# UltimateSoftware/surge

Hardware: AMD Instinct MI355X
Metric: events/sec replayed (higher is better)
Workload: dtype int32/int64 adds + bit-copied f64

## Files before the change

surge_amd/csrc/ingest_decoder.hip:

```cpp
#include <cstdio>
#include <cstdlib>

#include "ingest_decoder_internal.h"

using namespace surge::ingest;
using namespace surge::ingest::host;

namespace {

struct DecoderOptions {
  int push_streams = 3;
  bool push_streams_pinned = false, normal_priority = false, block_waits = true, weak_hash = false;
  int64_t poll_ns = 10000;
};

DecoderOptions read_options() {
  DecoderOptions o;
  if (const char* v = std::getenv("SURGE_INGEST_PUSH_STREAMS")) {
    o.push_streams = std::atoi(v);
    o.push_streams_pinned = true;
  }
  o.push_streams = o.push_streams < 1 ? 1 : (o.push_streams > kSlots ? kSlots : o.push_streams);
  if (const char* v = std::getenv("SURGE_INGEST_PUSH_PRIORITY")) o.normal_priority = std::strcmp(v, "normal") == 0;
  if (const char* v = std::getenv("SURGE_INGEST_WAIT")) {
    o.block_waits = std::strcmp(v, "spin") != 0;
    if (std::strcmp(v, "poll") != 0) o.poll_ns = 0;
  }
  if (o.poll_ns > 0)
    if (const char* u = std::getenv("SURGE_INGEST_POLL_US")) o.poll_ns = std::atoll(u) > 0 ? std::atoll(u) * 1000 : o.poll_ns;
  if (const char* v = std::getenv("SURGE_INGEST_DEBUG_WEAK_HASH")) o.weak_hash = v[0] == '1';
  return o;
}

int32_t create_streams_and_events(surge_device_decoder* d, const DecoderOptions& o) {
  d->push_streams_pinned = o.push_streams_pinned;
  for (int i = 0; i < o.push_streams; ++i) {
    int least = 0, greatest = 0;
    if (!o.normal_priority && hipDeviceGetStreamPriorityRange(&least, &greatest) == hipSuccess && least != greatest)
      DCHK(d, hipStreamCreateWithPriority(&d->push_streams[i], hipStreamNonBlocking, least));
    else
      DCHK(d, hipStreamCreateWithFlags(&d->push_streams[i], hipStreamNonBlocking));
    d->n_push_streams = d->n_push_active = i + 1;
  }
  for (PushSlot& s : d->slots) {
    DCHK(d, hipEventCreateWithFlags(&s.done, hipEventDisableTiming));
    DCHK(d, hipEventCreateWithFlags(&s.released, hipEventDisableTiming));
    DCHK(d, s.d_err.reserve(sizeof(ErrorCell), false, d->stream));
  }
  DCHK(d, hipEventCreateWithFlags(&d->ready, hipEventDisableTiming));
  DCHK(d, hipEventCreateWithFlags(&d->consumed, hipEventDisableTiming));
  return OK;
}

int32_t upload_template(surge_device_decoder* d, const surge_event_json_template* tmpl) {
  static EvjDevice ev;
  static std::mutex ev_mu;
  std::lock_guard<std::mutex> lk(ev_mu);
  std::memset(&ev, 0, sizeof(ev));
  ev.n_types = tmpl->n_types;
  auto intern = [&](const char* name) -> uint8_t {
// ... 70 lines not shown
    *rc = refuse_poisoned(d);
    return nullptr;
  }
  PushSlot* s = nullptr;
  {
    std::lock_guard<std::mutex> lk(d->mu);
    if (d->n_pending < kSlots) s = &d->slots[(d->head + d->n_pending) % kSlots];
    if (s) s->stream = d->push_streams[d->push_seq++ % (uint64_t)d->n_push_active];
  }
  if (!s) *rc = dfail(d, SURGE_E_STATE, "every push slot holds an unfinished push: call surge_device_decoder_push_finish first");
  return s;
}

int32_t await_release(surge_device_decoder* d, PushSlot& s) {
  if (!s.released_valid) return OK;
  DCHK(d, hipStreamWaitEvent(s.stream, s.released, 0));
  s.released_valid = false;
  return OK;
}

int32_t commit_slot(surge_device_decoder* d, PushSlot& s) {
  DCHK(d, hipEventRecord(s.done, s.stream));
  s.busy = true;
  std::lock_guard<std::mutex> lk(d->mu);
  ++d->n_pending;
  return OK;
}

template <typename Stage1>
int32_t enqueue_push(surge_device_decoder* d, Stage1 stage1) {
  int32_t rc = OK;
  PushSlot* s = claim_slot(d, &rc);
  if (!s) return rc;
  rc = await_release(d, *s);
  if (rc != OK) return rc;
  rc = stage1(*s);
  if (rc != OK) {
    (void)hipStreamSynchronize(s->stream);
    return rc;
  }
  return commit_slot(d, *s);
}

int32_t finish_oldest(surge_device_decoder* d, bool wait) {
  PushSlot* sp;
  {
    std::lock_guard<std::mutex> lk(d->mu);
    if (d->n_pending == 0) sp = nullptr;
    else sp = &d->slots[d->head];
  }
  if (!sp) return dfail(d, SURGE_E_STATE, "push_finish without a pending push_async");
  PushSlot& s = *sp;
  const int32_t rc = stage2(d, s, wait);
  if (rc != OK) {
    (void)hipStreamSynchronize(s.stream);
    (void)hipStreamSynchronize(d->stream);
    s.released_valid = false;
  }
  s.busy = false;
  std::lock_guard<std::mutex> lk(d->mu);
  d->head = (d->head + 1) % kSlots;
  --d->n_pending;
  return rc;
}

void* pinned_alloc(size_t n) {
  void* p = nullptr;
  return hipHostMalloc(&p, n, hipHostMallocDefault) == hipSuccess ? p : nullptr;
}
// ... 27 lines not shown
  return decoder_create(device_id, hip_stream, tmpl, false, out);
}

int32_t surge_device_decoder_create_states(int32_t device_id, void* hip_stream, surge_device_decoder** out) {
  return decoder_create(device_id, hip_stream, nullptr, true, out);
}

int32_t surge_device_decoder_destroy(surge_device_decoder* d) {
  if (!d) return OK;
#ifdef SURGE_EXPERIMENTS
  std::fprintf(stderr, "[surge experiments] decoder: %lld pushes, %lld batches chained by the one-lane walk after the parallel recognition declined\n", (long long)d->pushes,
               (long long)d->chain_fallbacks);
#endif
  DeviceScope scope(d->device);
  (void)hipStreamSynchronize(d->stream);
  for (int i = 0; i < d->n_push_streams; ++i) {
    (void)hipStreamSynchronize(d->push_streams[i]);
    (void)hipStreamDestroy(d->push_streams[i]);
  }
  for (PushSlot& s : d->slots) {
    if (s.done) (void)hipEventDestroy(s.done);
    if (s.released) (void)hipEventDestroy(s.released);
  }
  if (d->ready) (void)hipEventDestroy(d->ready);
  if (d->consumed) (void)hipEventDestroy(d->consumed);
  if (d->sleeper) (void)hipEventDestroy(d->sleeper);
  delete d;
  return OK;
}

int32_t surge_device_decoder_push_parts_floored_async(surge_device_decoder* d, int32_t n_parts, const uint8_t* const* bytes, const surge_batch_section* const* sections,
                                                      const int64_t* n_sections, int64_t n_floors, const surge_section_floor* floors) {
  if (!d) return refuse_null_decoder();
  if (n_parts < 0 || (n_parts > 0 && (!bytes || !sections || !n_sections)) || n_floors < 0 || (n_floors > 0 && !floors)) return dfail(d, E_INVALID, "bad argument");
  DeviceScope scope(d->device);
  return enqueue_push(d, [&](PushSlot& s) { return stage1_wire(d, s, n_parts, bytes, sections, n_sections, n_floors, floors); });
// ... 166 lines not shown
```

surge_amd/csrc/ingest_decoder_internal.h:

```cpp
#pragma once

#include <sys/prctl.h>
#include <time.h>

#include <atomic>
#include <cstring>
#include <mutex>
#include <new>
#include <string>
#include <utility>
#include <vector>

#include "../../include/surge_ingest.h"
#include "../../include/surge_replay.h"
#include "ingest_device.h"

namespace surge {
namespace ingest {
namespace host __attribute__((visibility("hidden"))) {

constexpr int32_t OK = 0, E_INVALID = -1, E_DEVICE = -3, E_NOMEM = -4, E_UNSUPPORTED = -5;

struct Buf {
  void* p = nullptr;
  size_t cap = 0;
  Buf() = default;
  Buf(const Buf&) = delete;
  Buf& operator=(const Buf&) = delete;
  Buf(Buf&& o) noexcept : p(o.p), cap(o.cap) { o.p = nullptr; o.cap = 0; }
  Buf& operator=(Buf&& o) noexcept {
// ... 10 lines not shown
    if (e != hipSuccess) return e;
    if (keep && p && cap) {
      e = hipMemcpyAsync(fresh, p, cap, hipMemcpyDeviceToDevice, stream);
      if (e == hipSuccess) e = hipStreamSynchronize(stream);
      if (e != hipSuccess) { (void)hipFree(fresh); return e; }
    }
    if (p) (void)hipFree(p);
    p = fresh;
    cap = want;
    return hipSuccess;
  }
  void release() { if (p) (void)hipFree(p); p = nullptr; cap = 0; }
};

struct PushSlot {
  Buf lz4_blocks, lz4_sizes, lz4_nseq, lz4_seq, lz4_cls;
  Buf sn_blocks, sn_sizes, sn_nseq, sn_seq, sn_cls;
  Buf d_bytes, d_sections, rec_a, rec_b, rec_c, meta, ev_tmp, f64_list, d_err;
  void* pinned = nullptr;
  size_t pinned_cap = 0;
  std::vector<Section> h_secs;
  Lz4Plan lz4;
  Lz4Plan snappy;
  int64_t snappy_host_sections = 0;
  std::vector<CrcSpan> h_crc;
  Buf crc_spans;
  std::vector<int64_t> h_floors;
  Buf d_floors;
  ErrorCell h_err;
  hipStream_t stream = nullptr;
  hipEvent_t done = nullptr;
  hipEvent_t released = nullptr;
  bool released_valid = false;
  int64_t n_rec = 0;
  uint64_t seed = 0;
  bool busy = false, wire = false;
  ~PushSlot() { if (pinned) (void)hipHostFree(pinned); }
};
constexpr int kSlots = 5;

struct ReadsState {
  struct Lookup { Buf ids, off, idx; } lookup;
  struct Order {
    Buf idx;
    int64_t keys = -1, passes = 0;
  } order;
// ... 61 lines not shown
  bool json = false;
  bool states = false;
  bool continued = false;
  bool keep_strings = false;
  std::mutex mu;
  std::atomic<bool> poisoned{false};
  std::string err;
  Buf d_tmpl, d_ptab;
  surge_event_json_template h_tmpl;
  PushSlot slots[kSlots];
  hipStream_t push_streams[kSlots] = {nullptr, nullptr, nullptr, nullptr, nullptr};
  int n_push_streams = 0;
  int n_push_active = 0;
  bool push_streams_pinned = false;
  uint64_t push_seq = 0;
  int head = 0;
  std::atomic<int> n_pending{0};
  Buf first, first_scan, keep, keep_pos, temp;
  Buf vlen, vscan, val_src, long_runs;
  Buf st_status, st_spans;
  Buf t_slots, arena, key_off, key_hash;
  uint64_t t_cap = 0;
  std::atomic<uint64_t> seed{0};
  int64_t n_keys = 0, arena_bytes = 0;
  Buf r_agg, r_ev, r_off;
  Buf r_val, r_val_off;
  int64_t val_bytes = 0;
  int64_t n_records = 0;
  int64_t state_loads = 0;
  uint64_t events_from_push = 0;
// ... 78 lines not shown
}

inline hipError_t wait_stream(surge_device_decoder* d, hipStream_t st) {
  if (!d->block_waits) return hipStreamSynchronize(st);
  hipError_t e = hipEventRecord(d->sleeper, st);
  if (e != hipSuccess || d->poll_ns <= 0) return e != hipSuccess ? e : hipEventSynchronize(d->sleeper);
  const int slack = prctl(PR_GET_TIMERSLACK, 0, 0, 0, 0);
  if (slack > 1000) (void)prctl(PR_SET_TIMERSLACK, 1000ul, 0, 0, 0);
  const timespec nap{0, (long)d->poll_ns};
  while ((e = hipEventQuery(d->sleeper)) == hipErrorNotReady) (void)nanosleep(&nap, nullptr);
  (void)hipGetLastError();
  if (slack > 1000) (void)prctl(PR_SET_TIMERSLACK, (unsigned long)slack, 0, 0, 0);
  return e;
}

int32_t stage1_wire(surge_device_decoder* d, PushSlot& s, int32_t n_parts, const uint8_t* const* bytes, const surge_batch_section* const* sections,
                    const int64_t* n_sections, int64_t n_floors, const surge_section_floor* floors);
int32_t stage1_records(surge_device_decoder* d, PushSlot& s, const uint8_t* keys, const int64_t* key_off, const uint8_t* values, const int64_t* value_off,
                       const int64_t* offsets, int64_t n);
int32_t stage2(surge_device_decoder* d, PushSlot& s, bool wait);
int32_t merge_event_strings(surge_device_decoder* d);
int32_t merge_state_strings(surge_device_decoder* d, surge_replay_handle* h, const surge_json_template* tmpl);

}
}
}
```

surge_amd/csrc/ingest_device.h:

```cpp
#pragma once

#include <hip/hip_runtime.h>
#include <stdint.h>

#include <vector>

#include "../../include/surge_ingest.h"
#include "f64_parse.h"

namespace surge {
namespace ingest {

enum : uint32_t {
  RS_OK = 0,
  RS_SKIP = 1,
  RS_NULL = 2,
  RS_MALFORMED = 3,
  RS_JSON = 4,
  RS_TYPE = 5,
  RS_FIELD = 6,
  RS_SIZE = 7,
  RS_F64_HOST = 8,
  RS_COLLISION = 9,
  RS_EMPTY_VALUE = 10,
// ... 150 lines not shown
  int64_t n_keys, arena_bytes;
};

struct InternScratch {
  unsigned long long *first, *first_scan;
  uint32_t *keep, *keep_pos;
  void* temp;
  size_t temp_bytes;
};

hipError_t launch_crc(const uint8_t* bytes, const CrcSpan* spans, int32_t n_spans, ErrorCell* err, hipStream_t st);

Lz4Route lz4_plan_section(Lz4Plan& plan, const uint8_t* frame, int64_t frame_len, int64_t src_off, int32_t section, int64_t* area_off,
                          std::vector<uint8_t>& host_out);
Lz4ScratchBytes lz4_scratch_bytes(const Lz4Plan& plan);
hipError_t launch_lz4(const Lz4Plan& plan, const uint8_t* bytes, uint8_t* area, const Lz4Block* d_blocks, Lz4Work w, Section* sections, ErrorCell* err, hipStream_t st);

hipError_t launch_lz4_exec(const uint8_t* bytes, uint8_t* area, const Lz4Block* d_blocks, int64_t n_blocks, Lz4Work w, hipStream_t st);

Lz4Route snappy_plan_section(Lz4Plan& plan, const uint8_t* sec, int64_t len, int64_t src_off, int32_t section, int64_t* area_off, std::vector<uint8_t>& host_out,
                             const char** why);
hipError_t launch_snappy(const Lz4Plan& plan, const uint8_t* bytes, uint8_t* area, const Lz4Block* d_blocks, Lz4Work w, Section* sections, ErrorCell* err, hipStream_t st);

hipError_t launch_sections(const uint8_t* bytes, const Section* sections, int64_t n_sections, int32_t max_recs, uint64_t seed, JsonCtx jc, RecMeta* meta,
                           uint4* ev_tmp, uint32_t* f64_host_list, ErrorCell* err, const int64_t* floors, hipStream_t st);
hipError_t launch_records(const uint8_t* bytes, const int64_t* key_off, const int64_t* val_off, const int64_t* offsets, int64_t val_base, int64_t n_rec,
                          uint64_t seed, JsonCtx jc, RecMeta* meta, uint4* ev_tmp, uint32_t* f64_host_list, ErrorCell* err, hipStream_t st);

hipError_t intern_temp_bytes(int64_t n_rec, size_t* bytes, hipStream_t st);
void launch_table_build(const KeyTable& k, hipStream_t st);
// ... 81 lines not shown
```

surge_amd/csrc/ingest_lz4.hip:

```cpp
#include <new>

#include "ingest_device.h"

namespace surge {
namespace ingest {
namespace {

constexpr int kLz4BlockMax = 65536;
struct Lz4Window {
  const uint8_t* in;
  int32_t n_in, wbase;
  uint32_t win;
  int lane;
  __device__ void refill(int32_t at) {
    wbase = at;
    const int32_t pos = at + 4 * lane;
    uint32_t v = 0;
    if (pos + 4 <= n_in) {
      v = (uint32_t)in[pos] | ((uint32_t)in[pos + 1] << 8) | ((uint32_t)in[pos + 2] << 16) | ((uint32_t)in[pos + 3] << 24);
    } else {
      for (int k = 0; k < 4; ++k)
        if (pos + k < n_in) v |= (uint32_t)in[pos + k] << (8 * k);
    }
    win = v;
// ... 442 lines not shown
  n.seq = (size_t)(plan.n_seq + 1) * 8;
  n.cls = (size_t)(kLz4Classes + 1) * (nb + 1) * 4;
  return n;
}

hipError_t launch_lz4_exec(const uint8_t* bytes, uint8_t* area, const Lz4Block* d_blocks, int64_t nb, Lz4Work w, hipStream_t st) {
  for (int c = 0; c <= kLz4Classes; ++c) {
    const int32_t cap = c < kLz4Classes ? kLz4ClassCapHost[c] : 0;
    const size_t lds = cap ? (size_t)cap + (size_t)kLz4Map * 2 : 0;
    const int64_t resident = 256ll * (lds ? (int64_t)(160 * 1024 / lds) : 16);
    hipLaunchKernelGGL(lz4_exec_kernel, dim3((unsigned)(nb < resident ? nb : resident)), dim3(64), lds, st, bytes, area, d_blocks, (int32_t)nb, w, c, cap);
  }
  return hipGetLastError();
}

hipError_t launch_lz4(const Lz4Plan& plan, const uint8_t* bytes, uint8_t* area, const Lz4Block* d_blocks, Lz4Work w, Section* sections, ErrorCell* err,
                      hipStream_t st) {
  const int64_t nb = (int64_t)plan.blocks.size();
  if (nb == 0) return hipSuccess;
  w.cls_list = w.cls_count + (kLz4Classes + 1);
  const hipError_t e = hipMemsetAsync(w.cls_count, 0, (kLz4Classes + 1) * 4, st);
  if (e != hipSuccess) return e;
  const int32_t parse_caps[3] = {6656, 16384 + 64, kLz4BlockMax + 64};
  for (int c = 0; c < 3; ++c)
    hipLaunchKernelGGL(lz4_parse_kernel, dim3((unsigned)nb), dim3(64), (size_t)parse_caps[c], st, bytes, area, d_blocks, (int32_t)nb, w, sections, err,
                       c == 0 ? -1 : parse_caps[c - 1], parse_caps[c]);
  (void)launch_lz4_exec(bytes, area, d_blocks, nb, w, st);
  bool any_one_pass = false;
  for (const Lz4Block& b : plan.blocks) any_one_pass = any_one_pass || b.seq_off < 0;
  if (any_one_pass) {
    const unsigned grid = (unsigned)(nb < 8192 ? nb : 8192);
    const int32_t caps[3] = {16384, 32768, kLz4BlockMax};
    for (int c = 0; c < 3; ++c)
      hipLaunchKernelGGL(lz4_block_kernel, dim3(grid), dim3(64), (size_t)caps[c], st, bytes, area, d_blocks, nb, w.state, c, caps[c], sections, err);
  }
  return hipGetLastError();
}
// ... 4 lines not shown
```

surge_amd/csrc/ingest_snappy.hip:

```cpp
#include <new>

#include "ingest_device.h"
#include "snappy_block.h"

namespace surge {
namespace ingest {
namespace {

constexpr int32_t kSnappyChunkMax = 65536;
constexpr int kSnappyParseClasses = 4;
constexpr int32_t kSnappyParseCap[kSnappyParseClasses] = {10240, 20480, 40960, 81920};
constexpr int32_t kSnappyStagePad = 80;
constexpr int32_t kSnappyStageMax = kSnappyParseCap[kSnappyParseClasses - 1] - 15 - kSnappyStagePad;
constexpr int32_t kSnappyShortLiteral = 16;

__device__ __forceinline__ int32_t wave_inclusive_sum(int32_t v, int lane) {
#pragma unroll
  for (int d = 1; d < 64; d <<= 1) {
    const int32_t u = __shfl_up(v, d, 64);
    if (lane >= d) v += u;
  }
  return v;
}

// ... 156 lines not shown
    host_out.resize(ex + (size_t)total);
    int64_t got = 0;
    st = sn::frame_decompress(sec, len, host_out.data() + ex, total, &got);
    if (st == sn::SN_OK) return LZ4_ON_HOST;
    host_out.resize(ex);
  }
  *why = sn::status_name(st);
  return st == sn::SN_TOO_LARGE ? LZ4_TOO_LARGE : LZ4_BAD_FRAME;
}

hipError_t launch_snappy(const Lz4Plan& plan, const uint8_t* bytes, uint8_t* area, const Lz4Block* d_blocks, Lz4Work w, Section* sections, ErrorCell* err,
                         hipStream_t st) {
  const int64_t nb = (int64_t)plan.blocks.size();
  if (nb == 0) return hipSuccess;
  w.cls_list = w.cls_count + (kLz4Classes + 1);
  const hipError_t e = hipMemsetAsync(w.cls_count, 0, (kLz4Classes + 1) * 4, st);
  if (e != hipSuccess) return e;
  for (int c = 0; c < kSnappyParseClasses; ++c)
    hipLaunchKernelGGL(snappy_parse_kernel, dim3((unsigned)nb), dim3(64), (size_t)kSnappyParseCap[c], st, bytes, area, d_blocks, (int32_t)nb, w, sections, err,
                       c == 0 ? -1 : kSnappyParseCap[c - 1], kSnappyParseCap[c]);
  return launch_lz4_exec(bytes, area, d_blocks, nb, w, st);
}

}
}
```

surge_amd/csrc/ingest_stage1.hip:

```cpp
#include <chrono>
#include <cstdio>
#include <cstdlib>

#include "ingest_decoder_internal.h"

using namespace surge::ingest;
using namespace surge::ingest::host;

namespace {

int32_t slot_scratch(surge_device_decoder* d, PushSlot& s, int64_t n_rec) {
  const size_t R = (size_t)n_rec;
  DCHK(d, s.meta.reserve(R * sizeof(RecMeta), false, s.stream));
  if (!d->states) DCHK(d, s.ev_tmp.reserve(R * 16, false, s.stream));
  if (!d->states) DCHK(d, s.f64_list.reserve(R * 4, false, s.stream));
  static const ErrorCell kZero{~0ull, 0u, 0u, ~0u, ~0u, 0u, ~0u};
  DCHK(d, hipMemcpyAsync(s.d_err.p, &kZero, sizeof(kZero), hipMemcpyHostToDevice, s.stream));
  return OK;
}

int32_t slot_pinned(surge_device_decoder* d, PushSlot& s, size_t bytes) {
  if (bytes <= s.pinned_cap) return OK;
  if (s.pinned) (void)hipHostFree(s.pinned);
  s.pinned = nullptr;
  s.pinned_cap = 0;
  bytes += bytes / 4 + 65536;
  DCHK(d, hipHostMalloc(&s.pinned, bytes, hipHostMallocDefault));
  s.pinned_cap = bytes;
  return OK;
}

int32_t dbg_decode() {
// ... 26 lines not shown
};

struct WireLayout {
  struct Part {
    int64_t lo, len, dev;
    bool in_place;
  };
  std::vector<Part> parts;
  std::vector<uint8_t> extra;
  int64_t total_sections = 0, n_rec = 0, n_raw = 0;
  int32_t max_recs = 0;
  int64_t area_base() const { return (n_raw + (int64_t)extra.size() + 15) & ~15ll; }
};

struct SlotNeeds {
  size_t bytes, sections, crc_spans, floors, pinned;
  int64_t n_rec;
  Lz4ScratchBytes lz4, snappy;
};

size_t pad16(size_t n) { return (n + 15) & ~(size_t)15; }

constexpr int64_t kSnappyMark = -(1ll << 62);

int32_t layout_sections(surge_device_decoder* d, PushSlot& s, int32_t n_parts, const surge_batch_section* const* sections, const int64_t* n_sections, WireLayout& L) {
  try {
    s.h_secs.resize((size_t)L.total_sections);
    L.parts.resize((size_t)n_parts);
  } catch (const std::bad_alloc&) {
    return dfail(d, E_NOMEM, "out of host memory");
  }
  int64_t at = 0;
  for (int32_t p = 0; p < n_parts; ++p) {
    int64_t lo = INT64_MAX, hi = 0;
// ... 82 lines not shown
  } catch (const std::bad_alloc&) {
    return dfail(d, E_NOMEM, "out of host memory");
  }
  if (s.lz4.blocks.size() >= (1ull << 31)) return dfail(d, E_UNSUPPORTED, "more than 2^31 LZ4 blocks in one push: push fewer sections at a time");
  if (s.snappy.blocks.size() >= (1ull << 31)) return dfail(d, E_UNSUPPORTED, "more than 2^31 snappy chunks in one push: push fewer sections at a time");
  for (Section& sc : s.h_secs) {
    if (sc.byte_off <= kSnappyMark) sc.byte_off = L.area_base() + s.lz4.area + (kSnappyMark - sc.byte_off);
    else if (sc.byte_off < 0) sc.byte_off = L.area_base() + (-1 - sc.byte_off);
  }
  return OK;
}

SlotNeeds slot_needs(const PushSlot& s, const uint8_t* const* bytes, WireLayout& L) {
  SlotNeeds n;
  n.bytes = (size_t)(L.area_base() + s.lz4.area + s.snappy.area) + 64;
  n.sections = sizeof(Section) * s.h_secs.size();
  n.crc_spans = sizeof(CrcSpan) * s.h_crc.size();
  n.n_rec = L.n_rec;
  n.lz4 = lz4_scratch_bytes(s.lz4);
  n.snappy = lz4_scratch_bytes(s.snappy);
  n.floors = 8 * s.h_floors.size();
  n.pinned = pad16(L.extra.size()) + n.sections + n.lz4.blocks + pad16(n.snappy.blocks) + pad16(n.crc_spans) + pad16(n.floors) + 64;
  for (size_t p = 0; p < L.parts.size(); ++p) {
    WireLayout::Part& part = L.parts[p];
    if (part.len == 0) continue;
    hipPointerAttribute_t attr;
    part.in_place = hipPointerGetAttributes(&attr, bytes[p] + part.lo) == hipSuccess && attr.type == hipMemoryTypeHost;
    (void)hipGetLastError();
    if (!part.in_place) n.pinned += pad16((size_t)part.len);
  }
  return n;
}

int32_t size_slot(surge_device_decoder* d, PushSlot& t, const SlotNeeds& n) {
  const size_t per_event = d->states ? 0 : (size_t)n.n_rec;
  const std::pair<Buf*, size_t> device[] = {{&t.d_bytes, n.bytes}, {&t.d_sections, n.sections}, {&t.meta, (size_t)n.n_rec * sizeof(RecMeta)}, {&t.ev_tmp, per_event * 16},
                                            {&t.f64_list, per_event * 4}, {&t.crc_spans, n.crc_spans}, {&t.d_floors, n.floors}, {&t.lz4_blocks, n.lz4.blocks}, {&t.lz4_sizes, n.lz4.state},
                                            {&t.lz4_nseq, n.lz4.n_seq}, {&t.lz4_seq, n.lz4.seq}, {&t.lz4_cls, n.lz4.cls}, {&t.sn_blocks, n.snappy.blocks},
                                            {&t.sn_sizes, n.snappy.state}, {&t.sn_nseq, n.snappy.n_seq}, {&t.sn_seq, n.snappy.seq}, {&t.sn_cls, n.snappy.cls}};
  for (const auto& b : device) DCHK(d, b.first->reserve(b.second, false, t.stream));
  return slot_pinned(d, t, n.pinned);
}

void warm_idle_slots(surge_device_decoder* d, PushSlot& s, const SlotNeeds& n) {
  if (d->slots_sized) return;
  d->slots_sized = true;
  {
    std::lock_guard<std::mutex> lk(d->mu);
    if (d->n_pending != 0) return;
  }
  for (PushSlot& t : d->slots)
    if (&t != &s && !t.busy && !t.released_valid && size_slot(d, t, n) != OK) (void)hipGetLastError();
}

int32_t stage_and_copy(surge_device_decoder* d, PushSlot& s, const uint8_t* const* bytes, const WireLayout& L) {
  hipStream_t st = s.stream;
  size_t staged = 0;
  auto stage = [&](const void* src, size_t len) -> const uint8_t* {
    uint8_t* at = (uint8_t*)s.pinned + staged;
    std::memcpy(at, src, len);
    staged += pad16(len);
    return at;
  };
  for (size_t p = 0; p < L.parts.size(); ++p) {
    const WireLayout::Part& part = L.parts[p];
    if (part.len == 0) continue;
    const uint8_t* src = bytes[p] + part.lo;
    if (!part.in_place) src = stage(src, (size_t)part.len);
    DCHK(d, hipMemcpyAsync((uint8_t*)s.d_bytes.p + part.dev, src, (size_t)part.len, hipMemcpyHostToDevice, st));
  }
  if (!L.extra.empty()) DCHK(d, hipMemcpyAsync((uint8_t*)s.d_bytes.p + L.n_raw, stage(L.extra.data(), L.extra.size()), L.extra.size(), hipMemcpyHostToDevice, st));
  const size_t sec_bytes = sizeof(Section) * s.h_secs.size(), crc_bytes = sizeof(CrcSpan) * s.h_crc.size(), blk_bytes = sizeof(Lz4Block) * s.lz4.blocks.size();
  DCHK(d, hipMemcpyAsync(s.d_sections.p, stage(s.h_secs.data(), sec_bytes), sec_bytes, hipMemcpyHostToDevice, st));
  if (crc_bytes) DCHK(d, hipMemcpyAsync(s.crc_spans.p, stage(s.h_crc.data(), crc_bytes), crc_bytes, hipMemcpyHostToDevice, st));
  if (blk_bytes) DCHK(d, hipMemcpyAsync(s.lz4_blocks.p, stage(s.lz4.blocks.data(), blk_bytes), blk_bytes, hipMemcpyHostToDevice, st));
  const size_t sn_bytes = sizeof(Lz4Block) * s.snappy.blocks.size();
  if (sn_bytes) DCHK(d, hipMemcpyAsync(s.sn_blocks.p, stage(s.snappy.blocks.data(), sn_bytes), sn_bytes, hipMemcpyHostToDevice, st));
  const size_t floor_bytes = 8 * s.h_floors.size();
  if (floor_bytes) DCHK(d, hipMemcpyAsync(s.d_floors.p, stage(s.h_floors.data(), floor_bytes), floor_bytes, hipMemcpyHostToDevice, st));
  return OK;
}

int32_t expand_floors(surge_device_decoder* d, PushSlot& s, int64_t total_sections, int64_t n_floors, const surge_section_floor* floors) {
  s.h_floors.clear();
  if (n_floors == 0) return OK;
  if (d->states) return dfail(d, SURGE_E_STATE, "a state decoder reads its topic from the beginning: floors belong to an events decoder");
  try {
    s.h_floors.assign((size_t)total_sections, INT64_MIN);
  } catch (const std::bad_alloc&) {
    return dfail(d, E_NOMEM, "out of host memory");
  }
  for (int64_t i = 0; i < n_floors; ++i) {
    if (floors[i].section < 0 || floors[i].section >= total_sections) return dfail(d, E_INVALID, "a floor names section " + std::to_string(floors[i].section) + ": the push has " + std::to_string(total_sections));
    int64_t& f = s.h_floors[(size_t)floors[i].section];
// ... 16 lines not shown
  s.n_rec = 0;
  s.wire = true;
  s.snappy.clear();
  s.snappy_host_sections = 0;
  if (L.total_sections >= (1ll << 31)) return dfail(d, E_UNSUPPORTED, "more than 2^31 batches in one push");
  int32_t rc = expand_floors(d, s, L.total_sections, n_floors, floors);
  if (rc != OK || L.total_sections == 0) return rc;
  rc = layout_sections(d, s, n_parts, sections, n_sections, L);
  if (rc != OK || L.n_rec == 0) return rc;
  if (L.n_rec >= (1ll << 32) - 1) return dfail(d, E_UNSUPPORTED, "more than 2^32 - 2 records in one push: push fewer sections at a time");
  rc = plan_frames(d, s, n_parts, bytes, sections, n_sections, L);
  if (rc != OK) return rc;
  laps.lap("walk sections");
  const SlotNeeds needs = slot_needs(s, bytes, L);
  warm_idle_slots(d, s, needs);
  rc = size_slot(d, s, needs);
  if (rc == OK) rc = slot_scratch(d, s, L.n_rec);
  if (rc == OK) laps.lap("reserve");
  if (rc == OK) rc = stage_and_copy(d, s, bytes, L);
  if (rc != OK) return rc;
  hipStream_t st = s.stream;
  const uint8_t* dby = (const uint8_t*)s.d_bytes.p;
  Section* dsec = (Section*)s.d_sections.p;
  ErrorCell* derr = (ErrorCell*)s.d_err.p;
  if (!s.h_crc.empty()) DCHK(d, launch_crc(dby, (const CrcSpan*)s.crc_spans.p, (int32_t)s.h_crc.size(), derr, st));
  laps.lap("copies");
  Lz4Work w{dbg_decode() / 10, (int32_t*)s.lz4_sizes.p, (int32_t*)s.lz4_nseq.p, (uint2*)s.lz4_seq.p, (int32_t*)s.lz4_cls.p, nullptr};
  DCHK(d, launch_lz4(s.lz4, dby, (uint8_t*)s.d_bytes.p + L.area_base(), (const Lz4Block*)s.lz4_blocks.p, w, dsec, derr, st));
  laps.lap("lz4 launches");
  Lz4Work ws{0, (int32_t*)s.sn_sizes.p, (int32_t*)s.sn_nseq.p, (uint2*)s.sn_seq.p, (int32_t*)s.sn_cls.p, nullptr};
  DCHK(d, launch_snappy(s.snappy, dby, (uint8_t*)s.d_bytes.p + L.area_base() + s.lz4.area, (const Lz4Block*)s.sn_blocks.p, ws, dsec, derr, st));
  laps.lap("snappy launches");
  const JsonCtx jc = json_ctx(d, dbg_decode() % 10);
  DCHK(d, launch_sections(dby, dsec, L.total_sections, L.max_recs, seed, jc, (RecMeta*)s.meta.p, (uint4*)s.ev_tmp.p, (uint32_t*)s.f64_list.p, derr,
                          s.h_floors.empty() ? nullptr : (const int64_t*)s.d_floors.p, st));
  laps.lap("section launches");
  s.n_rec = L.n_rec;
  s.seed = seed;
  return OK;
}

int32_t surge::ingest::host::stage1_records(surge_device_decoder* d, PushSlot& s, const uint8_t* keys, const int64_t* key_off, const uint8_t* values,
                                            const int64_t* value_off, const int64_t* offsets, int64_t n) {
  s.n_rec = 0;
  s.wire = false;
  const uint64_t seed = d->seed.load();
  if (n == 0) return OK;
  if (n >= (1ll << 32) - 1) return dfail(d, E_UNSUPPORTED, "more than 2^32 - 2 records in one push");
  const int64_t kb = key_off[n] - key_off[0], vb = value_off[n] - value_off[0];
  if (kb < 0 || vb < 0 || (kb > 0 && !keys) || (vb > 0 && !values)) return dfail(d, E_INVALID, "bad key / value spans");
  for (int64_t i = 0; i < n; ++i)
    if (key_off[i + 1] < key_off[i] || value_off[i + 1] < value_off[i]) return dfail(d, E_INVALID, "key_off / value_off must not decrease (record " + std::to_string(i) + ")");
  hipStream_t st = s.stream;
  const size_t n_bytes = (size_t)(kb + vb), off_bytes = (size_t)(n + 1) * 8;
  const size_t stage = n_bytes + 2 * off_bytes + (offsets ? (size_t)n * 8 : 0) + 64;
  DCHK(d, s.d_bytes.reserve(n_bytes + 16, false, st));
  DCHK(d, s.rec_a.reserve(off_bytes, false, st));
  DCHK(d, s.rec_b.reserve(off_bytes, false, st));
  DCHK(d, s.rec_c.reserve((size_t)n * 8 + 8, false, st));
  {
    int32_t rc = slot_scratch(d, s, n);
    if (rc == OK) rc = slot_pinned(d, s, stage);
    if (rc != OK) return rc;
  }
  uint8_t* pin = (uint8_t*)s.pinned;
  if (kb) std::memcpy(pin, keys + key_off[0], (size_t)kb);
  if (vb) std::memcpy(pin + kb, values + value_off[0], (size_t)vb);
  int64_t* p_ko = (int64_t*)(pin + ((n_bytes + 7) & ~(size_t)7));
  int64_t* p_vo = p_ko + (n + 1);
  int64_t* p_of = p_vo + (n + 1);
  for (int64_t i = 0; i <= n; ++i) { p_ko[i] = key_off[i] - key_off[0]; p_vo[i] = value_off[i] - value_off[0]; }
  if (offsets) std::memcpy(p_of, offsets, (size_t)n * 8);
  if (n_bytes) DCHK(d, hipMemcpyAsync(s.d_bytes.p, pin, n_bytes, hipMemcpyHostToDevice, st));
  DCHK(d, hipMemcpyAsync(s.rec_a.p, p_ko, off_bytes, hipMemcpyHostToDevice, st));
  DCHK(d, hipMemcpyAsync(s.rec_b.p, p_vo, off_bytes, hipMemcpyHostToDevice, st));
  if (offsets) DCHK(d, hipMemcpyAsync(s.rec_c.p, p_of, (size_t)n * 8, hipMemcpyHostToDevice, st));
  DCHK(d, launch_records((const uint8_t*)s.d_bytes.p, (const int64_t*)s.rec_a.p, (const int64_t*)s.rec_b.p, offsets ? (const int64_t*)s.rec_c.p : nullptr, kb, n, seed,
                         json_ctx(d, 0), (RecMeta*)s.meta.p, (uint4*)s.ev_tmp.p, (uint32_t*)s.f64_list.p, (ErrorCell*)s.d_err.p, st));
  s.n_rec = n;
  s.seed = seed;
  return OK;
}
```

surge_amd/csrc/ingest_stage2.hip:

```cpp
#include "ingest_decoder_internal.h"

using namespace surge::ingest;
using namespace surge::ingest::host;

namespace {

const char* const kWhyBad[] = {"", "", "has a null key or value (not an event)", "is malformed (a length runs past its record or batch)",
                               "is not the JSON object the event template describes", "names an event type the template does not know",
                               "lacks a field the template names, or the field is not the number it should be", "is not a 16-byte fixed event", "",
                               "collides with another key on its 64-bit hash",
                               "has an empty, non-null value under a key (a state record carries a value or the null of a tombstone)",
                               "is not the protobuf Event envelope the event template names ([aggregateId] [payload] and nothing else)",
                               "names another aggregateId in its envelope than the aggregate id of its key", "",
                               "lacks a string field its event class names (kept event strings), or that string is not a valid JSON string"};
static_assert(sizeof(kWhyBad) / sizeof(kWhyBad[0]) == RS_COUNT, "one text per record status");
const char* why_bad(uint32_t status) { return status < RS_COUNT ? kWhyBad[status] : "is bad"; }

bool malformed_record_offset(const PushSlot& s, int64_t rec, int64_t* offset) {
  size_t si = 0;
  while (si + 1 < s.h_secs.size() && s.h_secs[si + 1].rec_first <= rec) ++si;
  Section sec;
  std::vector<uint8_t> sb;
  if (si >= s.h_secs.size() || hipMemcpy(&sec, (const Section*)s.d_sections.p + si, sizeof(sec), hipMemcpyDeviceToHost) != hipSuccess || sec.byte_len <= 0 ||
      sec.byte_len >= (1ll << 31))
    return false;
  try { sb.resize((size_t)sec.byte_len); } catch (const std::bad_alloc&) { return false; }
  if (hipMemcpy(sb.data(), (const uint8_t*)s.d_bytes.p + sec.byte_off, sb.size(), hipMemcpyDeviceToHost) != hipSuccess) return false;
  size_t pos = 0;
  auto varlong = [&](int64_t* v) -> bool {
    uint64_t u = 0;
    for (int shift = 0; shift <= 63; shift += 7) {
      if (pos >= sb.size()) return false;
      const uint8_t b = sb[pos++];
      u |= (uint64_t)(b & 0x7f) << shift;
      if (!(b & 0x80)) { *v = (int64_t)(u >> 1) ^ -(int64_t)(u & 1); return true; }
    }
    return false;
  };
// ... 254 lines not shown
```

Before: 392.1 billion.

## Coalesce per-push metadata tables into one arena upload and add optional copy stream

The section, CRC span, LZ4/Snappy block and floor tables now live in one packed device arena. They are staged contiguously in pinned memory and sent with a single host-to-device copy instead of up to five separate ones. An optional dedicated copy stream, selected by an environment variable and off by default, can carry the uploads, error-cell reset and LZ4 class zeroing, with events ordering it against buffer growth and kernel launches. The intent is fewer copy submissions per push and, when enabled, overlap of copies with compute on the push streams, at the cost of extra events and synchronization complexity.

Result: no change. 392.8 billion, median of 2 (+0.2%).

```diff
diff --git a/surge_amd/csrc/ingest_decoder.hip b/surge_amd/csrc/ingest_decoder.hip
--- a/surge_amd/csrc/ingest_decoder.hip
+++ b/surge_amd/csrc/ingest_decoder.hip
@@ -12,6 +12,7 @@
   int push_streams = 3;
   bool push_streams_pinned = false, normal_priority = false, block_waits = true, weak_hash = false;
   int64_t poll_ns = 10000;
+  enum CopyStream { COPY_ON_PUSH_STREAM, COPY_STREAM_GREATEST, COPY_STREAM_NORMAL } copy_stream = COPY_ON_PUSH_STREAM;
 };
 
 DecoderOptions read_options() {
@@ -29,6 +30,10 @@
   if (o.poll_ns > 0)
     if (const char* u = std::getenv("SURGE_INGEST_POLL_US")) o.poll_ns = std::atoll(u) > 0 ? std::atoll(u) * 1000 : o.poll_ns;
   if (const char* v = std::getenv("SURGE_INGEST_DEBUG_WEAK_HASH")) o.weak_hash = v[0] == '1';
+  if (const char* v = std::getenv("SURGE_INGEST_COPY_STREAM"))
+    o.copy_stream = std::strcmp(v, "1") == 0        ? DecoderOptions::COPY_STREAM_GREATEST
+                    : std::strcmp(v, "normal") == 0 ? DecoderOptions::COPY_STREAM_NORMAL
+                                                    : DecoderOptions::COPY_ON_PUSH_STREAM;
   return o;
 }
 
@@ -42,8 +47,19 @@
       DCHK(d, hipStreamCreateWithFlags(&d->push_streams[i], hipStreamNonBlocking));
     d->n_push_streams = d->n_push_active = i + 1;
   }
+  if (o.copy_stream != DecoderOptions::COPY_ON_PUSH_STREAM) {
+    int least = 0, greatest = 0;
+    if (o.copy_stream == DecoderOptions::COPY_STREAM_GREATEST && hipDeviceGetStreamPriorityRange(&least, &greatest) == hipSuccess && least != greatest) {
+      DCHK(d, hipStreamCreateWithPriority(&d->copy_stream, hipStreamNonBlocking, greatest));
+      d->copy_priority = greatest;
+    } else {
+      DCHK(d, hipStreamCreateWithFlags(&d->copy_stream, hipStreamNonBlocking));
+    }
+  }
   for (PushSlot& s : d->slots) {
     DCHK(d, hipEventCreateWithFlags(&s.done, hipEventDisableTiming));
+    DCHK(d, hipEventCreateWithFlags(&s.copied, hipEventDisableTiming));
+    DCHK(d, hipEventCreateWithFlags(&s.sized, hipEventDisableTiming));
     DCHK(d, hipEventCreateWithFlags(&s.released, hipEventDisableTiming));
     DCHK(d, s.d_err.reserve(sizeof(ErrorCell), false, d->stream));
   }
@@ -144,7 +160,7 @@
 
 int32_t await_release(surge_device_decoder* d, PushSlot& s) {
   if (!s.released_valid) return OK;
-  DCHK(d, hipStreamWaitEvent(s.stream, s.released, 0));
+  DCHK(d, hipStreamWaitEvent(copy_stream_of(d, s), s.released, 0));
   s.released_valid = false;
   return OK;
 }
@@ -166,6 +182,7 @@
   if (rc != OK) return rc;
   rc = stage1(*s);
   if (rc != OK) {
+    if (d->copy_stream) (void)hipStreamSynchronize(d->copy_stream);
     (void)hipStreamSynchronize(s->stream);
     return rc;
   }
@@ -183,6 +200,7 @@
   PushSlot& s = *sp;
   const int32_t rc = stage2(d, s, wait);
   if (rc != OK) {
+    if (d->copy_stream) (void)hipStreamSynchronize(d->copy_stream);
     (void)hipStreamSynchronize(s.stream);
     (void)hipStreamSynchronize(d->stream);
     s.released_valid = false;
@@ -240,12 +258,16 @@
 #endif
   DeviceScope scope(d->device);
   (void)hipStreamSynchronize(d->stream);
+  if (d->copy_stream) (void)hipStreamSynchronize(d->copy_stream);
   for (int i = 0; i < d->n_push_streams; ++i) {
     (void)hipStreamSynchronize(d->push_streams[i]);
     (void)hipStreamDestroy(d->push_streams[i]);
   }
+  if (d->copy_stream) (void)hipStreamDestroy(d->copy_stream);
   for (PushSlot& s : d->slots) {
     if (s.done) (void)hipEventDestroy(s.done);
+    if (s.copied) (void)hipEventDestroy(s.copied);
+    if (s.sized) (void)hipEventDestroy(s.sized);
     if (s.released) (void)hipEventDestroy(s.released);
   }
   if (d->ready) (void)hipEventDestroy(d->ready);
diff --git a/surge_amd/csrc/ingest_decoder_internal.h b/surge_amd/csrc/ingest_decoder_internal.h
--- a/surge_amd/csrc/ingest_decoder_internal.h
+++ b/surge_amd/csrc/ingest_decoder_internal.h
@@ -14,6 +14,7 @@
 #include "../../include/surge_ingest.h"
 #include "../../include/surge_replay.h"
 #include "ingest_device.h"
+#include "ingest_table_arena.h"
 
 namespace surge {
 namespace ingest {
@@ -54,9 +55,16 @@
 };
 
 struct PushSlot {
-  Buf lz4_blocks, lz4_sizes, lz4_nseq, lz4_seq, lz4_cls;
-  Buf sn_blocks, sn_sizes, sn_nseq, sn_seq, sn_cls;
-  Buf d_bytes, d_sections, rec_a, rec_b, rec_c, meta, ev_tmp, f64_list, d_err;
+  Buf lz4_sizes, lz4_nseq, lz4_seq, lz4_cls;
+  Buf sn_sizes, sn_nseq, sn_seq, sn_cls;
+  Buf d_bytes, rec_a, rec_b, rec_c, meta, ev_tmp, f64_list, d_err;
+  Buf tables;
+  TableArena tab;
+  Section* d_sections() const { return tab.at<Section>(tables.p, TAB_SECTIONS); }
+  const CrcSpan* d_crc_spans() const { return tab.at<CrcSpan>(tables.p, TAB_CRC_SPANS); }
+  const Lz4Block* d_lz4_blocks() const { return tab.at<Lz4Block>(tables.p, TAB_LZ4_BLOCKS); }
+  const Lz4Block* d_sn_blocks() const { return tab.at<Lz4Block>(tables.p, TAB_SNAPPY_BLOCKS); }
+  const int64_t* d_floors() const { return tab.at<int64_t>(tables.p, TAB_FLOORS); }
   void* pinned = nullptr;
   size_t pinned_cap = 0;
   std::vector<Section> h_secs;
@@ -64,12 +72,12 @@
   Lz4Plan snappy;
   int64_t snappy_host_sections = 0;
   std::vector<CrcSpan> h_crc;
-  Buf crc_spans;
   std::vector<int64_t> h_floors;
-  Buf d_floors;
   ErrorCell h_err;
   hipStream_t stream = nullptr;
   hipEvent_t done = nullptr;
+  hipEvent_t copied = nullptr;
+  hipEvent_t sized = nullptr;
   hipEvent_t released = nullptr;
   bool released_valid = false;
   int64_t n_rec = 0;
@@ -161,6 +169,8 @@
   int n_push_active = 0;
   bool push_streams_pinned = false;
   uint64_t push_seq = 0;
+  hipStream_t copy_stream = nullptr;
+  int copy_priority = 0;
   int head = 0;
   std::atomic<int> n_pending{0};
   Buf first, first_scan, keep, keep_pos, temp;
@@ -269,6 +279,7 @@
   return e;
 }
 
+inline hipStream_t copy_stream_of(const surge_device_decoder* d, const PushSlot& s) { return d->copy_stream ? d->copy_stream : s.stream; }
 int32_t stage1_wire(surge_device_decoder* d, PushSlot& s, int32_t n_parts, const uint8_t* const* bytes, const surge_batch_section* const* sections,
                     const int64_t* n_sections, int64_t n_floors, const surge_section_floor* floors);
 int32_t stage1_records(surge_device_decoder* d, PushSlot& s, const uint8_t* keys, const int64_t* key_off, const uint8_t* values, const int64_t* value_off,
diff --git a/surge_amd/csrc/ingest_device.h b/surge_amd/csrc/ingest_device.h
--- a/surge_amd/csrc/ingest_device.h
+++ b/surge_amd/csrc/ingest_device.h
@@ -188,6 +188,7 @@
 Lz4Route lz4_plan_section(Lz4Plan& plan, const uint8_t* frame, int64_t frame_len, int64_t src_off, int32_t section, int64_t* area_off,
                           std::vector<uint8_t>& host_out);
 Lz4ScratchBytes lz4_scratch_bytes(const Lz4Plan& plan);
+hipError_t zero_lz4_classes(const Lz4Plan& plan, const Lz4Work& w, hipStream_t st);
 hipError_t launch_lz4(const Lz4Plan& plan, const uint8_t* bytes, uint8_t* area, const Lz4Block* d_blocks, Lz4Work w, Section* sections, ErrorCell* err, hipStream_t st);
 
 hipError_t launch_lz4_exec(const uint8_t* bytes, uint8_t* area, const Lz4Block* d_blocks, int64_t n_blocks, Lz4Work w, hipStream_t st);
diff --git a/surge_amd/csrc/ingest_lz4.hip b/surge_amd/csrc/ingest_lz4.hip
--- a/surge_amd/csrc/ingest_lz4.hip
+++ b/surge_amd/csrc/ingest_lz4.hip
@@ -480,13 +480,15 @@
   return hipGetLastError();
 }
 
+hipError_t zero_lz4_classes(const Lz4Plan& plan, const Lz4Work& w, hipStream_t st) {
+  return plan.blocks.empty() ? hipSuccess : hipMemsetAsync(w.cls_count, 0, (kLz4Classes + 1) * 4, st);
+}
+
 hipError_t launch_lz4(const Lz4Plan& plan, const uint8_t* bytes, uint8_t* area, const Lz4Block* d_blocks, Lz4Work w, Section* sections, ErrorCell* err,
                       hipStream_t st) {
   const int64_t nb = (int64_t)plan.blocks.size();
   if (nb == 0) return hipSuccess;
   w.cls_list = w.cls_count + (kLz4Classes + 1);
-  const hipError_t e = hipMemsetAsync(w.cls_count, 0, (kLz4Classes + 1) * 4, st);
-  if (e != hipSuccess) return e;
   const int32_t parse_caps[3] = {6656, 16384 + 64, kLz4BlockMax + 64};
   for (int c = 0; c < 3; ++c)
     hipLaunchKernelGGL(lz4_parse_kernel, dim3((unsigned)nb), dim3(64), (size_t)parse_caps[c], st, bytes, area, d_blocks, (int32_t)nb, w, sections, err,
diff --git a/surge_amd/csrc/ingest_snappy.hip b/surge_amd/csrc/ingest_snappy.hip
--- a/surge_amd/csrc/ingest_snappy.hip
+++ b/surge_amd/csrc/ingest_snappy.hip
@@ -194,8 +194,6 @@
   const int64_t nb = (int64_t)plan.blocks.size();
   if (nb == 0) return hipSuccess;
   w.cls_list = w.cls_count + (kLz4Classes + 1);
-  const hipError_t e = hipMemsetAsync(w.cls_count, 0, (kLz4Classes + 1) * 4, st);
-  if (e != hipSuccess) return e;
   for (int c = 0; c < kSnappyParseClasses; ++c)
     hipLaunchKernelGGL(snappy_parse_kernel, dim3((unsigned)nb), dim3(64), (size_t)kSnappyParseCap[c], st, bytes, area, d_blocks, (int32_t)nb, w, sections, err,
                        c == 0 ? -1 : kSnappyParseCap[c - 1], kSnappyParseCap[c]);
diff --git a/surge_amd/csrc/ingest_stage1.hip b/surge_amd/csrc/ingest_stage1.hip
--- a/surge_amd/csrc/ingest_stage1.hip
+++ b/surge_amd/csrc/ingest_stage1.hip
@@ -9,13 +9,38 @@
 
 namespace {
 
-int32_t slot_scratch(surge_device_decoder* d, PushSlot& s, int64_t n_rec) {
+int32_t reserve_on_slot(surge_device_decoder* d, PushSlot& s, Buf& b, size_t bytes, bool* grew) {
+  const size_t was = b.cap;
+  DCHK(d, b.reserve(bytes, false, s.stream));
+  *grew = *grew || b.cap != was;
+  return OK;
+}
+
+int32_t slot_scratch(surge_device_decoder* d, PushSlot& s, int64_t n_rec, bool* grew) {
   const size_t R = (size_t)n_rec;
-  DCHK(d, s.meta.reserve(R * sizeof(RecMeta), false, s.stream));
-  if (!d->states) DCHK(d, s.ev_tmp.reserve(R * 16, false, s.stream));
-  if (!d->states) DCHK(d, s.f64_list.reserve(R * 4, false, s.stream));
+  int32_t rc = reserve_on_slot(d, s, s.meta, R * sizeof(RecMeta), grew);
+  if (rc == OK && !d->states) rc = reserve_on_slot(d, s, s.ev_tmp, R * 16, grew);
+  if (rc == OK && !d->states) rc = reserve_on_slot(d, s, s.f64_list, R * 4, grew);
+  return rc;
+}
+
+int32_t order_behind_sizing(surge_device_decoder* d, PushSlot& s, bool grew) {
+  if (!grew || !d->copy_stream) return OK;
+  DCHK(d, hipEventRecord(s.sized, s.stream));
+  DCHK(d, hipStreamWaitEvent(d->copy_stream, s.sized, 0));
+  return OK;
+}
+
+int32_t copy_error_zero(surge_device_decoder* d, PushSlot& s, hipStream_t cs) {
   static const ErrorCell kZero{~0ull, 0u, 0u, ~0u, ~0u, 0u, ~0u};
-  DCHK(d, hipMemcpyAsync(s.d_err.p, &kZero, sizeof(kZero), hipMemcpyHostToDevice, s.stream));
+  DCHK(d, hipMemcpyAsync(s.d_err.p, &kZero, sizeof(kZero), hipMemcpyHostToDevice, cs));
+  return OK;
+}
+
+int32_t copies_done(surge_device_decoder* d, PushSlot& s) {
+  if (!d->copy_stream) return OK;
+  DCHK(d, hipEventRecord(s.copied, d->copy_stream));
+  DCHK(d, hipStreamWaitEvent(s.stream, s.copied, 0));
   return OK;
 }
 
@@ -72,10 +97,13 @@
 };
 
 struct SlotNeeds {
-  size_t bytes, sections, crc_spans, floors, pinned;
+  size_t bytes, pinned;
+  TableArena tables;
   int64_t n_rec;
   Lz4ScratchBytes lz4, snappy;
 };
+static_assert(alignof(Section) <= kTableAlign && alignof(CrcSpan) <= kTableAlign && alignof(Lz4Block) <= kTableAlign && alignof(int64_t) <= kTableAlign,
+              "a table's elements must be aligned where the arena puts them");
 
 size_t pad16(size_t n) { return (n + 15) & ~(size_t)15; }
 
@@ -188,13 +216,12 @@
 SlotNeeds slot_needs(const PushSlot& s, const uint8_t* const* bytes, WireLayout& L) {
   SlotNeeds n;
   n.bytes = (size_t)(L.area_base() + s.lz4.area + s.snappy.area) + 64;
-  n.sections = sizeof(Section) * s.h_secs.size();
-  n.crc_spans = sizeof(CrcSpan) * s.h_crc.size();
   n.n_rec = L.n_rec;
   n.lz4 = lz4_scratch_bytes(s.lz4);
   n.snappy = lz4_scratch_bytes(s.snappy);
-  n.floors = 8 * s.h_floors.size();
-  n.pinned = pad16(L.extra.size()) + n.sections + n.lz4.blocks + pad16(n.snappy.blocks) + pad16(n.crc_spans) + pad16(n.floors) + 64;
+  const size_t table_bytes[TAB_COUNT] = {sizeof(Section) * s.h_secs.size(), sizeof(CrcSpan) * s.h_crc.size(), n.lz4.blocks, n.snappy.blocks, 8 * s.h_floors.size()};
+  n.tables = table_arena_layout(table_bytes);
+  n.pinned = pad16(L.extra.size()) + n.tables.total + 64;
   for (size_t p = 0; p < L.parts.size(); ++p) {
     WireLayout::Part& part = L.parts[p];
     if (part.len == 0) continue;
@@ -206,13 +233,16 @@
   return n;
 }
 
-int32_t size_slot(surge_device_decoder* d, PushSlot& t, const SlotNeeds& n) {
+int32_t size_slot(surge_device_decoder* d, PushSlot& t, const SlotNeeds& n, bool* grew) {
   const size_t per_event = d->states ? 0 : (size_t)n.n_rec;
-  const std::pair<Buf*, size_t> device[] = {{&t.d_bytes, n.bytes}, {&t.d_sections, n.sections}, {&t.meta, (size_t)n.n_rec * sizeof(RecMeta)}, {&t.ev_tmp, per_event * 16},
-                                            {&t.f64_list, per_event * 4}, {&t.crc_spans, n.crc_spans}, {&t.d_floors, n.floors}, {&t.lz4_blocks, n.lz4.blocks}, {&t.lz4_sizes, n.lz4.state},
-                                            {&t.lz4_nseq, n.lz4.n_seq}, {&t.lz4_seq, n.lz4.seq}, {&t.lz4_cls, n.lz4.cls}, {&t.sn_blocks, n.snappy.blocks},
-                                            {&t.sn_sizes, n.snappy.state}, {&t.sn_nseq, n.snappy.n_seq}, {&t.sn_seq, n.snappy.seq}, {&t.sn_cls, n.snappy.cls}};
-  for (const auto& b : device) DCHK(d, b.first->reserve(b.second, false, t.stream));
+  const std::pair<Buf*, size_t> device[] = {{&t.d_bytes, n.bytes}, {&t.tables, n.tables.total}, {&t.meta, (size_t)n.n_rec * sizeof(RecMeta)}, {&t.ev_tmp, per_event * 16},
+                                            {&t.f64_list, per_event * 4}, {&t.lz4_sizes, n.lz4.state}, {&t.lz4_nseq, n.lz4.n_seq}, {&t.lz4_seq, n.lz4.seq},
+                                            {&t.lz4_cls, n.lz4.cls}, {&t.sn_sizes, n.snappy.state}, {&t.sn_nseq, n.snappy.n_seq}, {&t.sn_seq, n.snappy.seq},
+                                            {&t.sn_cls, n.snappy.cls}};
+  for (const auto& b : device) {
+    const int32_t rc = reserve_on_slot(d, t, *b.first, b.second, grew);
+    if (rc != OK) return rc;
+  }
   return slot_pinned(d, t, n.pinned);
 }
 
@@ -223,12 +253,12 @@
     std::lock_guard<std::mutex> lk(d->mu);
     if (d->n_pending != 0) return;
   }
+  bool grew = false;
   for (PushSlot& t : d->slots)
-    if (&t != &s && !t.busy && !t.released_valid && size_slot(d, t, n) != OK) (void)hipGetLastError();
-}
-
-int32_t stage_and_copy(surge_device_decoder* d, PushSlot& s, const uint8_t* const* bytes, const WireLayout& L) {
-  hipStream_t st = s.stream;
+    if (&t != &s && !t.busy && !t.released_valid && size_slot(d, t, n, &grew) != OK) (void)hipGetLastError();
+}
+
+int32_t stage_and_copy(surge_device_decoder* d, PushSlot& s, const uint8_t* const* bytes, const WireLayout& L, hipStream_t st) {
   size_t staged = 0;
   auto stage = [&](const void* src, size_t len) -> const uint8_t* {
     uint8_t* at = (uint8_t*)s.pinned + staged;
@@ -244,14 +274,11 @@
     DCHK(d, hipMemcpyAsync((uint8_t*)s.d_bytes.p + part.dev, src, (size_t)part.len, hipMemcpyHostToDevice, st));
   }
   if (!L.extra.empty()) DCHK(d, hipMemcpyAsync((uint8_t*)s.d_bytes.p + L.n_raw, stage(L.extra.data(), L.extra.size()), L.extra.size(), hipMemcpyHostToDevice, st));
-  const size_t sec_bytes = sizeof(Section) * s.h_secs.size(), crc_bytes = sizeof(CrcSpan) * s.h_crc.size(), blk_bytes = sizeof(Lz4Block) * s.lz4.blocks.size();
-  DCHK(d, hipMemcpyAsync(s.d_sections.p, stage(s.h_secs.data(), sec_bytes), sec_bytes, hipMemcpyHostToDevice, st));
-  if (crc_bytes) DCHK(d, hipMemcpyAsync(s.crc_spans.p, stage(s.h_crc.data(), crc_bytes), crc_bytes, hipMemcpyHostToDevice, st));
-  if (blk_bytes) DCHK(d, hipMemcpyAsync(s.lz4_blocks.p, stage(s.lz4.blocks.data(), blk_bytes), blk_bytes, hipMemcpyHostToDevice, st));
-  const size_t sn_bytes = sizeof(Lz4Block) * s.snappy.blocks.size();
-  if (sn_bytes) DCHK(d, hipMemcpyAsync(s.sn_blocks.p, stage(s.snappy.blocks.data(), sn_bytes), sn_bytes, hipMemcpyHostToDevice, st));
-  const size_t floor_bytes = 8 * s.h_floors.size();
-  if (floor_bytes) DCHK(d, hipMemcpyAsync(s.d_floors.p, stage(s.h_floors.data(), floor_bytes), floor_bytes, hipMemcpyHostToDevice, st));
+  uint8_t* const image = (uint8_t*)s.pinned + staged;
+  const void* const table[TAB_COUNT] = {s.h_secs.data(), s.h_crc.data(), s.lz4.blocks.data(), s.snappy.blocks.data(), s.h_floors.data()};
+  for (int t = 0; t < TAB_COUNT; ++t)
+    if (s.tab.has(t)) std::memcpy(image + s.tab.off[t], table[t], s.tab.bytes[t]);
+  if (s.tab.total) DCHK(d, hipMemcpyAsync(s.tables.p, image, s.tab.total, hipMemcpyHostToDevice, st));
   return OK;
 }
 
@@ -298,26 +325,35 @@
   laps.lap("walk sections");
   const SlotNeeds needs = slot_needs(s, bytes, L);
   warm_idle_slots(d, s, needs);
-  rc = size_slot(d, s, needs);
-  if (rc == OK) rc = slot_scratch(d, s, L.n_rec);
+  bool grew = false;
+  rc = size_slot(d, s, needs, &grew);
+  if (rc == OK) rc = slot_scratch(d, s, L.n_rec, &grew);
+  if (rc == OK) rc = order_behind_sizing(d, s, grew);
   if (rc == OK) laps.lap("reserve");
-  if (rc == OK) rc = stage_and_copy(d, s, bytes, L);
+  s.tab = needs.tables;
+  const hipStream_t cs = copy_stream_of(d, s);
+  Lz4Work w{dbg_decode() / 10, (int32_t*)s.lz4_sizes.p, (int32_t*)s.lz4_nseq.p, (uint2*)s.lz4_seq.p, (int32_t*)s.lz4_cls.p, nullptr};
+  Lz4Work ws{0, (int32_t*)s.sn_sizes.p, (int32_t*)s.sn_nseq.p, (uint2*)s.sn_seq.p, (int32_t*)s.sn_cls.p, nullptr};
+  if (rc == OK) rc = copy_error_zero(d, s, cs);
+  if (rc == OK) rc = stage_and_copy(d, s, bytes, L, cs);
   if (rc != OK) return rc;
+  DCHK(d, zero_lz4_classes(s.lz4, w, cs));
+  DCHK(d, zero_lz4_classes(s.snappy, ws, cs));
+  rc = copies_done(d, s);
+  if (rc != OK) return rc;
+  laps.lap("copies");
   hipStream_t st = s.stream;
   const uint8_t* dby = (const uint8_t*)s.d_bytes.p;
-  Section* dsec = (Section*)s.d_sections.p;
+  Section* dsec = s.d_sections();
   ErrorCell* derr = (ErrorCell*)s.d_err.p;
-  if (!s.h_crc.empty()) DCHK(d, launch_crc(dby, (const CrcSpan*)s.crc_spans.p, (int32_t)s.h_crc.size(), derr, st));
-  laps.lap("copies");
-  Lz4Work w{dbg_decode() / 10, (int32_t*)s.lz4_sizes.p, (int32_t*)s.lz4_nseq.p, (uint2*)s.lz4_seq.p, (int32_t*)s.lz4_cls.p, nullptr};
-  DCHK(d, launch_lz4(s.lz4, dby, (uint8_t*)s.d_bytes.p + L.area_base(), (const Lz4Block*)s.lz4_blocks.p, w, dsec, derr, st));
+  if (!s.h_crc.empty()) DCHK(d, launch_crc(dby, s.d_crc_spans(), (int32_t)s.h_crc.size(), derr, st));
+  laps.lap("crc launch");
+  DCHK(d, launch_lz4(s.lz4, dby, (uint8_t*)s.d_bytes.p + L.area_base(), s.d_lz4_blocks(), w, dsec, derr, st));
   laps.lap("lz4 launches");
-  Lz4Work ws{0, (int32_t*)s.sn_sizes.p, (int32_t*)s.sn_nseq.p, (uint2*)s.sn_seq.p, (int32_t*)s.sn_cls.p, nullptr};
-  DCHK(d, launch_snappy(s.snappy, dby, (uint8_t*)s.d_bytes.p + L.area_base() + s.lz4.area, (const Lz4Block*)s.sn_blocks.p, ws, dsec, derr, st));
+  DCHK(d, launch_snappy(s.snappy, dby, (uint8_t*)s.d_bytes.p + L.area_base() + s.lz4.area, s.d_sn_blocks(), ws, dsec, derr, st));
   laps.lap("snappy launches");
   const JsonCtx jc = json_ctx(d, dbg_decode() % 10);
-  DCHK(d, launch_sections(dby, dsec, L.total_sections, L.max_recs, seed, jc, (RecMeta*)s.meta.p, (uint4*)s.ev_tmp.p, (uint32_t*)s.f64_list.p, derr,
-                          s.h_floors.empty() ? nullptr : (const int64_t*)s.d_floors.p, st));
+  DCHK(d, launch_sections(dby, dsec, L.total_sections, L.max_recs, seed, jc, (RecMeta*)s.meta.p, (uint4*)s.ev_tmp.p, (uint32_t*)s.f64_list.p, derr, s.d_floors(), st));
   laps.lap("section launches");
   s.n_rec = L.n_rec;
   s.seed = seed;
@@ -338,13 +374,17 @@
   hipStream_t st = s.stream;
   const size_t n_bytes = (size_t)(kb + vb), off_bytes = (size_t)(n + 1) * 8;
   const size_t stage = n_bytes + 2 * off_bytes + (offsets ? (size_t)n * 8 : 0) + 64;
-  DCHK(d, s.d_bytes.reserve(n_bytes + 16, false, st));
-  DCHK(d, s.rec_a.reserve(off_bytes, false, st));
-  DCHK(d, s.rec_b.reserve(off_bytes, false, st));
-  DCHK(d, s.rec_c.reserve((size_t)n * 8 + 8, false, st));
+  const hipStream_t cs = copy_stream_of(d, s);
   {
-    int32_t rc = slot_scratch(d, s, n);
+    bool grew = false;
+    int32_t rc = reserve_on_slot(d, s, s.d_bytes, n_bytes + 16, &grew);
+    if (rc == OK) rc = reserve_on_slot(d, s, s.rec_a, off_bytes, &grew);
+    if (rc == OK) rc = reserve_on_slot(d, s, s.rec_b, off_bytes, &grew);
+    if (rc == OK) rc = reserve_on_slot(d, s, s.rec_c, (size_t)n * 8 + 8, &grew);
+    if (rc == OK) rc = slot_scratch(d, s, n, &grew);
+    if (rc == OK) rc = order_behind_sizing(d, s, grew);
     if (rc == OK) rc = slot_pinned(d, s, stage);
+    if (rc == OK) rc = copy_error_zero(d, s, cs);
     if (rc != OK) return rc;
   }
   uint8_t* pin = (uint8_t*)s.pinned;
@@ -355,10 +395,14 @@
   int64_t* p_of = p_vo + (n + 1);
   for (int64_t i = 0; i <= n; ++i) { p_ko[i] = key_off[i] - key_off[0]; p_vo[i] = value_off[i] - value_off[0]; }
   if (offsets) std::memcpy(p_of, offsets, (size_t)n * 8);
-  if (n_bytes) DCHK(d, hipMemcpyAsync(s.d_bytes.p, pin, n_bytes, hipMemcpyHostToDevice, st));
-  DCHK(d, hipMemcpyAsync(s.rec_a.p, p_ko, off_bytes, hipMemcpyHostToDevice, st));
-  DCHK(d, hipMemcpyAsync(s.rec_b.p, p_vo, off_bytes, hipMemcpyHostToDevice, st));
-  if (offsets) DCHK(d, hipMemcpyAsync(s.rec_c.p, p_of, (size_t)n * 8, hipMemcpyHostToDevice, st));
+  if (n_bytes) DCHK(d, hipMemcpyAsync(s.d_bytes.p, pin, n_bytes, hipMemcpyHostToDevice, cs));
+  DCHK(d, hipMemcpyAsync(s.rec_a.p, p_ko, off_bytes, hipMemcpyHostToDevice, cs));
+  DCHK(d, hipMemcpyAsync(s.rec_b.p, p_vo, off_bytes, hipMemcpyHostToDevice, cs));
+  if (offsets) DCHK(d, hipMemcpyAsync(s.rec_c.p, p_of, (size_t)n * 8, hipMemcpyHostToDevice, cs));
+  {
+    const int32_t rc = copies_done(d, s);
+    if (rc != OK) return rc;
+  }
   DCHK(d, launch_records((const uint8_t*)s.d_bytes.p, (const int64_t*)s.rec_a.p, (const int64_t*)s.rec_b.p, offsets ? (const int64_t*)s.rec_c.p : nullptr, kb, n, seed,
                          json_ctx(d, 0), (RecMeta*)s.meta.p, (uint4*)s.ev_tmp.p, (uint32_t*)s.f64_list.p, (ErrorCell*)s.d_err.p, st));
   s.n_rec = n;
diff --git a/surge_amd/csrc/ingest_stage2.hip b/surge_amd/csrc/ingest_stage2.hip
--- a/surge_amd/csrc/ingest_stage2.hip
+++ b/surge_amd/csrc/ingest_stage2.hip
@@ -21,7 +21,7 @@
   while (si + 1 < s.h_secs.size() && s.h_secs[si + 1].rec_first <= rec) ++si;
   Section sec;
   std::vector<uint8_t> sb;
-  if (si >= s.h_secs.size() || hipMemcpy(&sec, (const Section*)s.d_sections.p + si, sizeof(sec), hipMemcpyDeviceToHost) != hipSuccess || sec.byte_len <= 0 ||
+  if (si >= s.h_secs.size() || hipMemcpy(&sec, s.d_sections() + si, sizeof(sec), hipMemcpyDeviceToHost) != hipSuccess || sec.byte_len <= 0 ||
       sec.byte_len >= (1ll << 31))
     return false;
   try { sb.resize((size_t)sec.byte_len); } catch (const std::bad_alloc&) { return false; }
diff --git a/surge_amd/csrc/ingest_table_arena.h b/surge_amd/csrc/ingest_table_arena.h
--- /dev/null
+++ b/surge_amd/csrc/ingest_table_arena.h
@@ -0,0 +1,34 @@
+#pragma once
+
+#include <stddef.h>
+
+namespace surge {
+namespace ingest {
+
+enum TableId { TAB_SECTIONS = 0, TAB_CRC_SPANS = 1, TAB_LZ4_BLOCKS = 2, TAB_SNAPPY_BLOCKS = 3, TAB_FLOORS = 4, TAB_COUNT = 5 };
+
+constexpr size_t kTableAlign = 16;
+
+struct TableArena {
+  size_t off[TAB_COUNT] = {0, 0, 0, 0, 0};
+  size_t bytes[TAB_COUNT] = {0, 0, 0, 0, 0};
+  size_t total = 0;
+  bool has(int t) const { return bytes[t] != 0; }
+  template <typename T>
+  T* at(void* base, int t) const { return has(t) ? (T*)((unsigned char*)base + off[t]) : nullptr; }
+  template <typename T>
+  const T* at(const void* base, int t) const { return has(t) ? (const T*)((const unsigned char*)base + off[t]) : nullptr; }
+};
+
+inline TableArena table_arena_layout(const size_t bytes[TAB_COUNT]) {
+  TableArena a;
+  for (int t = 0; t < TAB_COUNT; ++t) {
+    a.off[t] = a.total;
+    a.bytes[t] = bytes[t];
+    a.total += (bytes[t] + (kTableAlign - 1)) & ~(kTableAlign - 1);
+  }
+  return a;
+}
+
+}
+}
```
